# Mingqj/DFU3D

Measured on AMD Instinct MI355X. Metric: pseudo-box frames/sec (34k pts, 6 cams), higher is better.
Workload: dtype f64; 1 GPU; configs[1] with depth back-projection on (dense): 64 synthetic frames/GPU/step, 34720-pt sweep, 6 cams x 1600x900 depth + 8 instance masks (one bit-packed 1-byte word per pixel), 30-40 objects/scene; views_per_launch_chunk=192, streams=2, parallelism=frames sharded x1

## Files before the change

### dfu3d_amd/_lib.py

```python
import ctypes
import os
import re

from . import _build

c_void_p = ctypes.c_void_p
c_i32 = ctypes.c_int32
c_i64 = ctypes.c_int64
c_u64 = ctypes.c_uint64
c_f64 = ctypes.c_double

HEADER = os.path.join(_build.INCLUDE, "dfu3d.h")


class BinGeom(ctypes.Structure):
    _fields_ = [
        ("vsize_r", c_f64), ("vsize_t", c_f64), ("vsize_p", c_f64),
        ("rmin_r", c_f64), ("rmin_t", c_f64), ("rmin_p", c_f64),
        ("grid_r", c_i32), ("grid_t", c_i32), ("grid_p", c_i32),
        ("t_lo", c_i32), ("t_n", c_i32), ("p_lo", c_i32), ("p_n", c_i32),
        ("max_points_per_voxel", c_i32), ("max_voxels", c_i32),
        ("theta_min", c_f64), ("z_max", c_f64), ("depth_min", c_f64),
    ]

# ... 64 lines not shown
                                     _P]),
    "dfu3d_ballquery_fuse_joint": (c_i32, [_P, _P, _P, _P, _P, _P, _P, c_f64, c_i32, c_i64, _P, _P,
                                     _P]),
    "dfu3d_range_cluster": (c_i32, [_P, _P, _P, _P, c_i32, c_f64, c_f64, _P, _P, _P, _P, c_i64,
                                    _P]),
    "dfu3d_points_in_boxes_mask": (c_i32, [_P, c_i32, c_i32, _P, c_i32, _P, _P]),
    "dfu3d_gt_database": (c_i32, [_P, _P, _P, _P, c_i32, _P, _P, c_i64, _P, _P, _P, _P]),
    "dfu3d_boxes_bev": (c_i32, [_P, c_i32, _P, c_i32, _P, c_i32, _P]),
    "dfu3d_nms_bev": (c_i32, [_P, c_i32, ctypes.c_float, _P, _P, _P, _P]),
    "dfu3d_nms_normal_bev": (c_i32, [_P, c_i32, ctypes.c_float, _P, _P, _P, _P]),
    "dfu3d_boxes_bev_paired": (c_i32, [_P, _P, c_i32, _P, c_i32, _P]),
    "dfu3d_rotate_iou_eval": (c_i32, [_P, c_i32, _P, c_i32, _P, c_i32, _P]),
    "dfu3d_eval_overlaps": (c_i32, [c_i32, c_i32, _P, _P, _P, _P, _P, _P, _P, _P, c_i64, _P]),
    "dfu3d_eval_match_scores": (c_i32, [c_i32, c_i32, c_i32] + [_P] * 15 + [c_i32, c_i64, _P, _P, _P]),
    "dfu3d_eval_match_stats": (c_i32, [c_i32, c_i32, c_i32] + [_P] * 15 + [c_i32, _P, _P, c_i32, c_i32, _P, _P, _P]),
    "dfu3d_workspace_bytes": (c_i64, [c_i32, ctypes.POINTER(Sizes)]),
    "dfu3d_chain_workspace_bytes": (c_i64, [ctypes.POINTER(ChainCfg)]),
    "dfu3d_chain_workspace_init": (c_i32, [ctypes.POINTER(ChainCfg), _P, _P]),
    "dfu3d_pseudo_boxes": (c_i32, [ctypes.POINTER(ChainCfg)] + [_P] * 20),
    "dfu3d_la_sampling": (c_i32, [_P, c_i32, _P, c_i32, ctypes.c_float, ctypes.c_float, _P, _P, _P, c_i64, _P]),
    "dfu3d_selftest_classify": (c_i32, [_P, c_i32, c_i32, _P, c_i32, c_i64, ctypes.c_uint64, c_f64, c_f64, _P, _P, _P]),
    "dfu3d_selftest_backproject": (c_i32, [_P, c_i32, c_i32, c_i64, ctypes.c_uint64, c_f64, c_f64, _P, _P, _P]),
    "dfu3d_lshape_fit_ws_doubles": (c_i64, [c_i64, c_i32]),
    "dfu3d_lshape_fit": (c_i32, [_P, _P, _P, _P, _P, _P, c_i32, c_i32, _P, _P, _P, _P, _P,
                                 c_i32, c_f64, c_f64, _P, _P, _P, c_i32, _P, _P, _P, _P, c_i64,
                                 _P]),
}

_LIB = None


class Dfu3dError(RuntimeError):
    pass


def header_symbols():
    text = open(HEADER).read()
    text = re.sub(r"/\*.*?\*/", "", text, flags=re.S)
    return sorted(set(re.findall(r"\b(dfu3d_[a-z0-9_]+)\s*\(", text)))


def header_version():
    return int(re.search(r"#define\s+DFU3D_VERSION\s+(\d+)", open(HEADER).read()).group(1))


def lib():
# ... 43 lines not shown
```

### dfu3d_amd/csrc/fit_stage.hip

```cpp
#include "common.hpp"

namespace {
__device__ __forceinline__ int rl_i(int v, int l) { return __builtin_amdgcn_readlane(v, l); }
__device__ __forceinline__ double rl_d(double v, int l) {
  return __hiloint2double(__builtin_amdgcn_readlane(__double2hiint(v), l), __builtin_amdgcn_readlane(__double2loint(v), l));
}

constexpr int CT = 512;
constexpr int GRP = 32;
constexpr int BLK = 32;
constexpr int PAIR_SMALL = 32;
constexpr int GU = 4;
constexpr int SMALL_N = 4096;
constexpr int LARGE_N = 61440;
constexpr int LARGE_GRP = LARGE_N / GRP;
constexpr int GRID_NC_SMALL = 4096;
constexpr int GRID_NC_LARGE = 12288;

struct ParI {
  int *p;
  bool global;
  __device__ __forceinline__ int load(int i) const {
    return __hip_atomic_load(p + i, __ATOMIC_RELAXED, __HIP_MEMORY_SCOPE_AGENT);
  }
// ... 781 lines not shown
    const int slot = atomicAdd(n_rows, 1);
    if (slot < cap_rows) {
      double *o = rows + (size_t)slot * DFU3D_ROW_DOUBLES;
      o[0] = (double)v; o[1] = (double)jinst; o[2] = (double)kc;
      o[3] = (double)inst_class[s]; o[4] = alpha;
      o[5] = (double)inst_box[s * 4 + 0]; o[6] = (double)inst_box[s * 4 + 1];
      o[7] = (double)inst_box[s * 4 + 2]; o[8] = (double)inst_box[s * 4 + 3];
      o[9] = height; o[10] = width; o[11] = length;
      o[12] = rx; o[13] = ry; o[14] = rz; o[15] = rotation;
      o[16] = (double)inst_score[s]; o[17] = (double)m;
      o[18] = thb; o[19] = c1min; o[20] = c2min; o[21] = c1max; o[22] = c2max;
      o[23] = (double)root;
    } else {
      atomicOr(status, DFU3D_ST_ROW_OVERFLOW);
    }
  }
}

struct FitWs {
  int *counters;
  double *dsc;
  int *big_list;
  double *big_cost;
  int cap_q, cap_big;
};
__host__ __device__ inline int fit_cap_q(int cap_rows) { return 2 * cap_rows + 64; }
__host__ __device__ inline FitWs fit_ws_view(double *ws, int cap_rows, int cap_big) {
  FitWs w;
  w.cap_q = fit_cap_q(cap_rows);
  w.cap_big = cap_big;
  w.counters = (int *)ws;
  w.dsc = ws + 2;
  w.big_list = (int *)(w.dsc + (size_t)8 * w.cap_q);
  w.big_cost = w.dsc + (size_t)8 * w.cap_q + (cap_big / 2 + 1);
  return w;
}

constexpr int GK = 512;

__device__ __forceinline__ int rank_in(const int *roots, int nk, int L) {
  int lo = 0, hi = nk - 1;
  while (lo < hi) {
    const int mid = (lo + hi) >> 1;
    if (roots[mid] < L) lo = mid + 1; else hi = mid;
  }
  return (roots[lo] == L) ? lo : -1;
}

constexpr int GGU = 4;
__global__ __launch_bounds__(FT) void k_fit_gather(
    const double *__restrict__ px, const double *__restrict__ py,
    const double *__restrict__ pz, const int *__restrict__ label,
    const long long *__restrict__ seg_base, const int *__restrict__ seg_cnt,
    double *__restrict__ gsx, double *__restrict__ gsy, int *__restrict__ sroot,
    uint32_t *__restrict__ status, double *__restrict__ fit_ws, int cap_rows, int cap_big) {
  __shared__ int s_roots[GK];
  __shared__ int s_cnt[FW][GK];
// ... 181 lines not shown
struct FitAcc {
  double s1, s2, q1, q2;
  int n1, n2;
  __device__ __forceinline__ void clear() { s1 = s2 = q1 = q2 = 0.0; n1 = n2 = 0; }
  __device__ __forceinline__ void add(double x, double y, double ct, double st, double a0, double a1, double b0, double b1) {
    const double c1 = x * ct + y * st;
    const double c2 = x * (-st) + y * ct;
    const double d1 = fmin(fabs(a1 - c1), fabs(c1 - a0));
    const double d2 = fmin(fabs(b1 - c2), fabs(c2 - b0));
    if (d1 < d2) { s1 += d1; q1 = fma(d1, d1, q1); n1++; } else { s2 += d2; q2 = fma(d2, d2, q2); n2++; }
  }
  __device__ __forceinline__ void wave_reduce() {
    s1 = wave_sum_d(s1); s2 = wave_sum_d(s2); q1 = wave_sum_d(q1); q2 = wave_sum_d(q2);
    n1 = wave_sum_i(n1); n2 = wave_sum_i(n2);
  }
  __device__ __forceinline__ double cost(double &mag) const {
    double V1 = 0.0, V2 = 0.0, M1 = 0.0, M2 = 0.0;
    if (n1) { const double mu = s1 / (double)n1; M1 = q1 / (double)n1; V1 = -(M1 - mu * mu); }
    if (n2) { const double mu = s2 / (double)n2; M2 = q2 / (double)n2; V2 = -(M2 - mu * mu); }
    mag = M1 + M2;
    return V1 + V2;
  }
};
__device__ __forceinline__ double wave_exact_cost(const double *mx, const double *my, int m, double ct, double st) {
  const int lane = lane_id();
  double a0 = INFINITY, a1 = -INFINITY, b0 = INFINITY, b1 = -INFINITY;
  for (int i = lane; i < m; i += 64) {
    const double x = mx[i], y = my[i];
    const double c1 = x * ct + y * st;
    const double c2 = x * (-st) + y * ct;
    a0 = fmin(a0, c1); a1 = fmax(a1, c1);
    b0 = fmin(b0, c2); b1 = fmax(b1, c2);
  }
  a0 = wave_min_d(a0); a1 = wave_max_d(a1);
  b0 = wave_min_d(b0); b1 = wave_max_d(b1);
  double s1 = 0.0, s2 = 0.0;
  int n1 = 0, n2 = 0;
  for (int i = lane; i < m; i += 64) {
    const double x = mx[i], y = my[i];
    const double c1 = x * ct + y * st;
    const double c2 = x * (-st) + y * ct;
    const double d1 = fmin(fabs(a1 - c1), fabs(c1 - a0));
    const double d2 = fmin(fabs(b1 - c2), fabs(c2 - b0));
    if (d1 < d2) { s1 += d1; n1++; } else { s2 += d2; n2++; }
  }
  s1 = wave_sum_d(s1); s2 = wave_sum_d(s2);
// ... 150 lines not shown
      const double c1 = x * cos_s + y * sin_s;
      const double c2 = x * (-sin_s) + y * cos_s;
      a0 = c1; a1 = c1; b0 = c2; b1 = c2;
    }
    a0 = wave_min_d(a0); a1 = wave_max_d(a1);
    b0 = wave_min_d(b0); b1 = wave_max_d(b1);
    if (lane == 0) {
      const int s = (int)d[0], kc = (int)d[1], root = (int)d[2];
      const int v = s / max_inst, jinst = s - v * max_inst;
      emit_box(thb, sin_s, cos_s, a0, a1, b0, b1, d[5], s, v, jinst, kc, root, m, calib, inst_class,
               inst_is_car, inst_box, inst_score, car_aspect_max, cap_rows, rows, n_rows, status);
    }
  }
}

__global__ __launch_bounds__(FT, 8) void k_fit_medium(
    const double *__restrict__ gsx, const double *__restrict__ gsy, int max_inst,
    const ViewCalib *__restrict__ calib, const int *__restrict__ inst_class,
    const int *__restrict__ inst_is_car, const float *__restrict__ inst_box,
    const float *__restrict__ inst_score, int n_theta, double dtheta, double car_aspect_max,
    int cap_rows, double *__restrict__ rows, int *__restrict__ n_rows,
    uint32_t *__restrict__ status, double *__restrict__ fit_ws, int cap_big) {
  __shared__ double lx[LDS_MEMBERS], ly[LDS_MEMBERS];
  __shared__ double s_cost[MAXTH], s_mag[MAXTH], s_ct[MAXTH], s_st[MAXTH];
  __shared__ double s_ext[FW][4];
  const FitWs W = fit_ws_view(fit_ws, cap_rows, cap_big);
  const int nq = min(W.counters[0], W.cap_q);
  const int wave = threadIdx.x >> 6, lane = lane_id();
  if (threadIdx.x < MAXTH) {
    const double theta = (double)threadIdx.x * dtheta;
    s_ct[threadIdx.x] = cos(theta);
    s_st[threadIdx.x] = sin(theta);
  }
  __shared__ int s_item;
  while (true) {
    __syncthreads();
    if (wave == 0) {
      const int ticket = atomicAdd(&W.counters[3], 1);
      if (lane == 0) s_item = ticket >> 6;
    }
    __syncthreads();
    const int e = s_item;
    if (e >= nq) break;
    const double *d = W.dsc + (size_t)8 * e;
    const int m = (int)d[3];
    if (m <= 64 || m > LDS_MEMBERS) continue;
    __syncthreads();
    const long long P = (long long)d[4];
    for (int i = threadIdx.x; i < m; i += FT) { lx[i] = gsx[P + i]; ly[i] = gsy[P + i]; }
    __syncthreads();
    const double *mx = lx;
    const double *my = ly;
    for (int th0 = 2 * wave; th0 < n_theta; th0 += 2 * FW) {
      const int th1 = min(th0 + 1, n_theta - 1);
      const double ct0 = s_ct[th0], st0 = s_st[th0], ct1 = s_ct[th1], st1 = s_st[th1];
      double a0 = INFINITY, a1 = -INFINITY, b0 = INFINITY, b1 = -INFINITY;
      double e0 = INFINITY, e1 = -INFINITY, f0 = INFINITY, f1 = -INFINITY;
      for (int i = lane; i < m; i += 64) {
        const double x = mx[i], y = my[i];
        double c1 = x * ct0 + y * st0;
        double c2 = x * (-st0) + y * ct0;
        a0 = min_raw_d(a0, c1); a1 = max_raw_d(a1, c1);
        b0 = min_raw_d(b0, c2); b1 = max_raw_d(b1, c2);
        c1 = x * ct1 + y * st1;
        c2 = x * (-st1) + y * ct1;
        e0 = min_raw_d(e0, c1); e1 = max_raw_d(e1, c1);
        f0 = min_raw_d(f0, c2); f1 = max_raw_d(f1, c2);
      }
      a0 = wave_min_d(a0); a1 = wave_max_d(a1); b0 = wave_min_d(b0); b1 = wave_max_d(b1);
      e0 = wave_min_d(e0); e1 = wave_max_d(e1); f0 = wave_min_d(f0); f1 = wave_max_d(f1);
      FitAcc A, B;
      A.clear(); B.clear();
      for (int i = lane; i < m; i += 64) {
        const double x = mx[i], y = my[i];
        A.add(x, y, ct0, st0, a0, a1, b0, b1);
        B.add(x, y, ct1, st1, e0, e1, f0, f1);
      }
      A.wave_reduce(); B.wave_reduce();
      double magA, magB;
      const double cA = A.cost(magA), cB = B.cost(magB);
      if (lane == 0) { s_cost[th0] = cA; s_mag[th0] = magA; s_cost[th1] = cB; s_mag[th1] = magB; }
    }
    __syncthreads();
    double magmax = 0.0;
    for (int th = 0; th < n_theta; th++) { const double g = s_mag[th]; if (g > magmax) magmax = g; }
    const int best = wave_pick_heading(s_cost, n_theta, magmax, mx, my, m, s_ct, s_st);
    const double thb = (double)best * dtheta;
    const double sin_s = sin(thb), cos_s = cos(thb);
    {
      double a0 = INFINITY, a1 = -INFINITY, b0 = INFINITY, b1 = -INFINITY;
      for (int i = threadIdx.x; i < m; i += FT) {
        const double x = mx[i], y = my[i];
        const double c1 = x * cos_s + y * sin_s;
        const double c2 = x * (-sin_s) + y * cos_s;
        a0 = fmin(a0, c1); a1 = fmax(a1, c1);
        b0 = fmin(b0, c2); b1 = fmax(b1, c2);
      }
      a0 = wave_min_d(a0); a1 = wave_max_d(a1);
      b0 = wave_min_d(b0); b1 = wave_max_d(b1);
      if (lane == 0) { s_ext[wave][0] = a0; s_ext[wave][1] = a1; s_ext[wave][2] = b0; s_ext[wave][3] = b1; }
    }
    __syncthreads();
    if (threadIdx.x == 0) {
      double c1min = s_ext[0][0], c1max = s_ext[0][1], c2min = s_ext[0][2], c2max = s_ext[0][3];
      for (int w = 1; w < FW; w++) {
        c1min = fmin(c1min, s_ext[w][0]); c1max = fmax(c1max, s_ext[w][1]);
        c2min = fmin(c2min, s_ext[w][2]); c2max = fmax(c2max, s_ext[w][3]);
      }
      const int s = (int)d[0], kc = (int)d[1], root = (int)d[2];
      const int v = s / max_inst, jinst = s - v * max_inst;
      emit_box(thb, sin_s, cos_s, c1min, c1max, c2min, c2max, d[5], s, v, jinst, kc, root, m, calib,
               inst_class, inst_is_car, inst_box, inst_score, car_aspect_max, cap_rows, rows,
               n_rows, status);
    }
  }
}

constexpr int BIGC_T = 512, BIGC_WAVES = BIGC_T / 64, BIGC_HPW = 2, BIGC_HB = BIGC_WAVES * BIGC_HPW;
constexpr int BIGC_CH = 4096;
constexpr int BIGC_LONG = 16384, BIGC_MID = 6144;
__global__ __launch_bounds__(BIGC_T) void k_fit_big_cost(const double *__restrict__ gsx,
                                                         const double *__restrict__ gsy, int n_theta,
                                                         double dtheta, double *__restrict__ fit_ws,
                                                         int cap_rows, int cap_big) {
  __shared__ double lx[BIGC_CH], ly[BIGC_CH];
  __shared__ double s_ct[MAXTH], s_st[MAXTH];
  __shared__ int s_item;
  const FitWs W = fit_ws_view(fit_ws, cap_rows, cap_big);
  const int nbig = min(W.counters[1], cap_big);
  if (nbig == 0) return;
  if (threadIdx.x < MAXTH) {
    const double theta = (double)threadIdx.x * dtheta;
    s_ct[threadIdx.x] = cos(theta);
    s_st[threadIdx.x] = sin(theta);
  }
  const int wave = threadIdx.x >> 6, lane = lane_id();
  const int nb = (n_theta + BIGC_HB - 1) / BIGC_HB;
  const int items = nbig * nb;
  while (true) {
    __syncthreads();
    if (wave == 0) {
      const int ticket = atomicAdd(&W.counters[2], 1);
      if (lane == 0) s_item = ticket >> 6;
    }
    __syncthreads();
    const int ticket_item = s_item;
    if (ticket_item >= 3 * items) break;
    const int round = ticket_item / items;
    const int item = ticket_item - round * items;
    const int c = item / nb, tb = (item - c * nb) * BIGC_HB;
    const double *dsc = W.dsc + (size_t)8 * W.big_list[c];
    const int m = (int)dsc[3];
    if ((m > BIGC_LONG ? 0 : (m > BIGC_MID ? 1 : 2)) != round) continue;
    const double *mx = gsx + (long long)dsc[4], *my = gsy + (long long)dsc[4];
    int th[BIGC_HPW];
    double ct[BIGC_HPW], st[BIGC_HPW], nst[BIGC_HPW];
#pragma unroll
    for (int h = 0; h < BIGC_HPW; h++) {
      th[h] = tb + wave * BIGC_HPW + h;
      const int tc = min(th[h], n_theta - 1);
      ct[h] = s_ct[tc]; st[h] = s_st[tc]; nst[h] = -st[h];
    }
    double a0[BIGC_HPW], a1[BIGC_HPW], b0[BIGC_HPW], b1[BIGC_HPW];
#pragma unroll
    for (int h = 0; h < BIGC_HPW; h++) { a0[h] = INFINITY; a1[h] = -INFINITY; b0[h] = INFINITY; b1[h] = -INFINITY; }
    for (int c0 = 0; c0 < m; c0 += BIGC_CH) {
      const int cm = min(BIGC_CH, m - c0);
      __syncthreads();
      for (int i = threadIdx.x; i < cm; i += BIGC_T) { lx[i] = mx[c0 + i]; ly[i] = my[c0 + i]; }
      __syncthreads();
      for (int i = lane; i < cm; i += 64) {
        const double x = lx[i], y = ly[i];
#pragma unroll
        for (int h = 0; h < BIGC_HPW; h++) {
          const double c1 = x * ct[h] + y * st[h];
          const double c2 = x * nst[h] + y * ct[h];
          a0[h] = min_raw_d(a0[h], c1); a1[h] = max_raw_d(a1[h], c1);
          b0[h] = min_raw_d(b0[h], c2); b1[h] = max_raw_d(b1[h], c2);
        }
      }
    }
#pragma unroll
    for (int h = 0; h < BIGC_HPW; h++) {
      a0[h] = wave_min_d(a0[h]); a1[h] = wave_max_d(a1[h]);
      b0[h] = wave_min_d(b0[h]); b1[h] = wave_max_d(b1[h]);
    }
    FitAcc A[BIGC_HPW];
#pragma unroll
    for (int h = 0; h < BIGC_HPW; h++) A[h].clear();
    for (int c0 = 0; c0 < m; c0 += BIGC_CH) {
      const int cm = min(BIGC_CH, m - c0);
      __syncthreads();
      for (int i = threadIdx.x; i < cm; i += BIGC_T) { lx[i] = mx[c0 + i]; ly[i] = my[c0 + i]; }
      __syncthreads();
      for (int i = lane; i < cm; i += 64) {
        const double x = lx[i], y = ly[i];
#pragma unroll
        for (int h = 0; h < BIGC_HPW; h++) A[h].add(x, y, ct[h], st[h], a0[h], a1[h], b0[h], b1[h]);
      }
    }
#pragma unroll
    for (int h = 0; h < BIGC_HPW; h++) {
      A[h].wave_reduce();
      double mag;
      const double cst = A[h].cost(mag);
      if (lane == 0 && th[h] < n_theta) {
        W.big_cost[(size_t)c * MAXTH + th[h]] = cst;
        if (mag > 0.0) atomicMax((unsigned long long *)(W.dsc + (size_t)8 * W.big_list[c] + 7), (unsigned long long)__double_as_longlong(mag));
// ... 35 lines not shown
    const double c1 = x * cos_s + y * sin_s;
    const double c2 = x * (-sin_s) + y * cos_s;
    a0 = fmin(a0, c1); a1 = fmax(a1, c1);
    b0 = fmin(b0, c2); b1 = fmax(b1, c2);
  }
  a0 = wave_min_d(a0); a1 = wave_max_d(a1);
  b0 = wave_min_d(b0); b1 = wave_max_d(b1);
  if (lane == 0) { s_ext[wave][0] = a0; s_ext[wave][1] = a1; s_ext[wave][2] = b0; s_ext[wave][3] = b1; }
  __syncthreads();
  if (threadIdx.x == 0) {
    double c1min = s_ext[0][0], c1max = s_ext[0][1], c2min = s_ext[0][2], c2max = s_ext[0][3];
    for (int w = 1; w < FW; w++) {
      c1min = fmin(c1min, s_ext[w][0]); c1max = fmax(c1max, s_ext[w][1]);
      c2min = fmin(c2min, s_ext[w][2]); c2max = fmax(c2max, s_ext[w][3]);
    }
    const int v = s / max_inst, jinst = s - v * max_inst;
    emit_box(thb, sin_s, cos_s, c1min, c1max, c2min, c2max, zmax, s, v, jinst, kc, root, m, calib,
             inst_class, inst_is_car, inst_box, inst_score, car_aspect_max, cap_rows, rows, n_rows,
             status);
  }
  }
}

}

extern "C" int dfu3d_range_cluster(const double *px, const double *py, const int64_t *seg_base,
                                   const int32_t *seg_cnt, int32_t S, double R0, double Rd,
                                   int32_t *label, double *sx, double *sy, int32_t *si,
                                   int64_t pool_cap, void *stream) {
  DFU3D_CLEAR_STALE_ERROR();
  if (!px || !py || !seg_base || !seg_cnt || !label || !sx || !sy || !si) return DFU3D_EINVAL;
  if (S <= 0 || pool_cap <= 0 || !(R0 > 0.0) || !(Rd >= 0.0)) return DFU3D_EINVAL;
  hipLaunchKernelGGL((k_range_cluster_grid<GRID_NC_SMALL, 0, 1024>), dim3(CL_CLASSES * S), dim3(1024), 0,
                     (hipStream_t)stream, px, py, (const long long *)seg_base, seg_cnt, R0, Rd,
                     label, sx, sy, si, (long long)pool_cap, 0, 0x7FFFFFFF);
  DFU3D_LAUNCH_CHECK();
  hipLaunchKernelGGL((k_range_cluster_grid<GRID_NC_LARGE, GRID_NC_SMALL, 1024>), dim3(CL_CLASSES * S), dim3(1024), 0,
                     (hipStream_t)stream, px, py, (const long long *)seg_base, seg_cnt, R0, Rd,
                     label, sx, sy, si, (long long)pool_cap, 0, 0x7FFFFFFF);
  DFU3D_LAUNCH_CHECK();
  hipLaunchKernelGGL(k_range_cluster_small, dim3(S), dim3(CT), 0, (hipStream_t)stream, px, py,
                     (const long long *)seg_base, seg_cnt, R0, Rd, label, sx, sy, si,
                     (long long)pool_cap);
  DFU3D_LAUNCH_CHECK();
  hipLaunchKernelGGL(k_range_cluster_large, dim3(S), dim3(CT), 0, (hipStream_t)stream, px, py,
                     (const long long *)seg_base, seg_cnt, R0, Rd, label, sx, sy, si,
                     (long long)pool_cap);
  DFU3D_LAUNCH_CHECK();
  return DFU3D_OK;
}


extern "C" int64_t dfu3d_lshape_fit_ws_doubles(int64_t pool_cap, int32_t cap_rows) {
  if (pool_cap <= 0 || cap_rows <= 0) return DFU3D_EINVAL;
  const int64_t cap_big = pool_cap / LDS_MEMBERS + 1;
  return 2 + (int64_t)8 * fit_cap_q(cap_rows) + (cap_big / 2 + 1) + cap_big * MAXTH;
}

extern "C" int dfu3d_lshape_fit(const double *px, const double *py, const double *pz,
                                const int32_t *label, const int64_t *seg_base,
                                const int32_t *seg_cnt, int32_t S, int32_t max_inst,
                                const float *calib, const int32_t *inst_class,
                                const int32_t *inst_is_car, const float *inst_box,
                                const float *inst_score, int32_t n_theta, double dtheta,
                                double car_aspect_max, double *sx, double *sy, int32_t *sroot,
                                int32_t cap_rows, double *rows, int32_t *n_rows,
                                uint32_t *status, double *fit_ws, int64_t pool_cap,
                                void *stream) {
  DFU3D_CLEAR_STALE_ERROR();
  if (!px || !py || !pz || !label || !seg_base || !seg_cnt || !calib || !inst_class ||
      !inst_is_car || !inst_box || !inst_score || !sx || !sy || !sroot || !rows || !n_rows ||
      !status || !fit_ws)
    return DFU3D_EINVAL;
  if (S <= 0 || max_inst <= 0 || cap_rows <= 0 || n_theta <= 0 || pool_cap <= 0) return DFU3D_EINVAL;
  if (n_theta > MAXTH) return DFU3D_ERANGE;
  hipStream_t st = (hipStream_t)stream;
  const int cap_big = (int)(pool_cap / LDS_MEMBERS + 1);
  const ViewCalib *vc = (const ViewCalib *)calib;
  if (dfu3d_fill_small_async(fit_ws, 16, nullptr, 0, nullptr, 0, st) != hipSuccess) return DFU3D_ELAUNCH;
  hipLaunchKernelGGL(k_fit_gather, dim3(3 * S), dim3(FT), 0, st, px, py, pz, label,
                     (const long long *)seg_base, seg_cnt, sx, sy, sroot, status, fit_ws,
                     cap_rows, cap_big);
  DFU3D_LAUNCH_CHECK();
  const int cap_q = fit_cap_q(cap_rows);
  const int g_tiny = cap_q / 4 + 1 < 2048 ? cap_q / 4 + 1 : 2048;
  hipLaunchKernelGGL(k_fit_tiny, dim3(g_tiny), dim3(256), 0, st, sx, sy, max_inst, vc, inst_class,
                     inst_is_car, inst_box, inst_score, n_theta, dtheta, car_aspect_max, cap_rows,
                     rows, n_rows, status, fit_ws, cap_big);
  DFU3D_LAUNCH_CHECK();
  hipLaunchKernelGGL(k_fit_medium, dim3(cap_q < 2048 ? cap_q : 2048), dim3(FT), 0, st, sx, sy, max_inst,
                     vc, inst_class, inst_is_car, inst_box, inst_score, n_theta, dtheta,
                     car_aspect_max, cap_rows, rows, n_rows, status, fit_ws, cap_big);
  DFU3D_LAUNCH_CHECK();
  const long long bi = (long long)cap_big * ((n_theta + BIGC_HB - 1) / BIGC_HB);
  const int g2 = (int)(bi < 2048 ? bi : 2048);
  hipLaunchKernelGGL(k_fit_big_cost, dim3(g2), dim3(BIGC_T), 0, st, sx, sy, n_theta, dtheta,
                     fit_ws, cap_rows, cap_big);
  DFU3D_LAUNCH_CHECK();
  hipLaunchKernelGGL(k_fit_big_box, dim3(cap_big < 2048 ? cap_big : 2048), dim3(FT), 0, st, sx, sy, max_inst,
                     vc, inst_class, inst_is_car, inst_box, inst_score,
                     n_theta, dtheta, car_aspect_max, cap_rows, rows, n_rows, status, fit_ws,
                     cap_big);
  DFU3D_LAUNCH_CHECK();
  return DFU3D_OK;
}

extern "C" int dfu3d_version(void) { return DFU3D_VERSION; }

extern "C" const char *dfu3d_strerror(int code) {
  switch (code) {
    case DFU3D_OK: return "ok";
    case DFU3D_EINVAL: return "invalid argument";
    case DFU3D_ELAUNCH: return "kernel launch failed";
    case DFU3D_ERANGE: return "size exceeds a compiled-in limit";
    default: return "unknown error";
  }
// ... 2 lines not shown
```

### dfu3d_amd/stages.py

```python
import ctypes
import math

import numpy as np
from dataclasses import dataclass

import torch

from . import _lib
from ._lib import BinGeom, Dfu3dError

CALIB_FLOATS = 48
ROW_DOUBLES = 24
MAX_INST = 32

BP_BIN, BP_AMB, BP_MARK, BP_VOX, BP_REPAIR, BP_ALL = 1, 2, 4, 8, 16, 31
MASK_BYTES = 0
RF_SHADOW, RF_FLAGS, RF_RESOLVE, RF_COMPACT, RF_ALL = 1, 2, 4, 8, 15

ST_POOL_OVERFLOW = 1
ST_VOX_OVERFLOW = 2
ST_ROW_OVERFLOW = 4
ST_BIN_RANGE = 8
ST_VOX_PTS_OVERFLOW = 16
ST_VOXEL_RANGE = 32
# ... 476 lines not shown
    scratch = torch.zeros(SELFTEST_SCRATCH_BYTES // 4, dtype=torch.float32, device=device)
    out = torch.zeros(4, dtype=torch.int64, device=device)
    rc = _lib.lib().dfu3d_selftest_classify(_chk(cal, "calib", torch.float32, numel=CALIB_FLOATS), int(H), int(W),
                                            ctypes.byref(geom), int(key_axis), int(n), int(seed), float(d_lo),
                                            float(d_hi), _chk(scratch, "scratch", torch.float32),
                                            _chk(out, "out", torch.int64, numel=4), _stream())
    _lib.check(rc, "dfu3d_selftest_classify")
    t, u, w, k = out.cpu().tolist()
    return {"tried": t, "undecided": u, "wrong": w, "kept": k}


def selftest_backproject(calib_record, H, W, n, seed=1, d_lo=0.5, d_hi=120.0, device="cuda:0"):
    cal = torch.as_tensor(np.asarray(calib_record, np.float32).reshape(CALIB_FLOATS)).to(device).contiguous()
    scratch = torch.zeros(32, dtype=torch.float32, device=device)
    out = torch.zeros(1, dtype=torch.float64, device=device)
    rc = _lib.lib().dfu3d_selftest_backproject(_chk(cal, "calib", torch.float32, numel=CALIB_FLOATS), int(H), int(W),
                                               int(n), int(seed), float(d_lo), float(d_hi),
                                               _chk(scratch, "scratch", torch.float32, numel=32),
                                               _chk(out, "out", torch.float64, numel=1), _stream())
    _lib.check(rc, "dfu3d_selftest_backproject")
    return float(out.item())


def range_cluster(px, py, seg_base, seg_cnt, S, R0, Rd, label, pool_cap, sx=None, sy=None, si=None):
    dev = px.device
    sx = sx if sx is not None else torch.empty(pool_cap, dtype=torch.float64, device=dev)
    sy = sy if sy is not None else torch.empty(pool_cap, dtype=torch.float64, device=dev)
    si = si if si is not None else torch.empty(3 * pool_cap, dtype=torch.int32, device=dev)
    rc = _lib.lib().dfu3d_range_cluster(
        _chk(px, "px", torch.float64, numel=pool_cap), _chk(py, "py", torch.float64, numel=pool_cap),
        _chk(seg_base, "seg_base", torch.int64, numel=S),
        _chk(seg_cnt, "seg_cnt", torch.int32, numel=S), S, float(R0), float(Rd),
        _chk(label, "label", torch.int32, numel=pool_cap),
        _chk(sx, "sx", torch.float64, numel=pool_cap), _chk(sy, "sy", torch.float64, numel=pool_cap),
        _chk(si, "si", torch.int32, numel=3 * pool_cap), pool_cap, _stream())
    _lib.check(rc, "dfu3d_range_cluster")


def lshape_fit(px, py, pz, label, seg_base, seg_cnt, S, max_inst, calib, inst_class,
               inst_is_car, inst_box, inst_score, n_theta, dtheta, car_aspect_max, sx, sy,
               sroot, cap_rows, rows, n_rows, status, pool_cap, fit_ws=None):
    nws = int(_lib.lib().dfu3d_lshape_fit_ws_doubles(pool_cap, cap_rows))
    if fit_ws is None:
        fit_ws = torch.empty(nws, dtype=torch.float64, device=px.device)
    if S % max_inst:
        raise Dfu3dError("S must be V*max_inst")
# ... 25 lines not shown
```

### include/dfu3d.h

```cpp
#ifndef DFU3D_H
#define DFU3D_H

#include <stddef.h>
#include <stdint.h>

#ifdef __cplusplus
extern "C" {
#endif

#define DFU3D_VERSION 150
#define DFU3D_CALIB_FLOATS 48
#define DFU3D_ROW_DOUBLES 24
#define DFU3D_TABLE_ENTRY_BYTES 28
#define DFU3D_MAX_INST 32

#define DFU3D_OK 0
#define DFU3D_EINVAL (-1)
#define DFU3D_ELAUNCH (-2)
#define DFU3D_ERANGE (-3)

#define DFU3D_ST_POOL_OVERFLOW 1u
#define DFU3D_ST_VOX_OVERFLOW 2u
#define DFU3D_ST_ROW_OVERFLOW 4u
#define DFU3D_ST_BIN_RANGE 8u
// ... 202 lines not shown
int dfu3d_selftest_classify(const float *calib, int32_t H, int32_t W, const dfu3d_bin_geom *geom,
                            int32_t key_axis, int64_t n, uint64_t seed, double d_lo, double d_hi,
                            void *scratch, uint64_t *out4, void *stream);
int dfu3d_selftest_backproject(const float *calib, int32_t H, int32_t W, int64_t n, uint64_t seed,
                               double d_lo, double d_hi, void *scratch64, double *out1, void *stream);

int dfu3d_range_cluster(const double *px, const double *py,
                        const int64_t *seg_base, const int32_t *seg_cnt,
                        int32_t S, double R0, double Rd, int32_t *label,
                        double *sx, double *sy, int32_t *si, int64_t pool_cap,
                        void *stream);

int64_t dfu3d_lshape_fit_ws_doubles(int64_t pool_cap, int32_t cap_rows);
int dfu3d_lshape_fit(const double *px, const double *py, const double *pz,
                     const int32_t *label, const int64_t *seg_base,
                     const int32_t *seg_cnt, int32_t S, int32_t max_inst,
                     const float *calib, const int32_t *inst_class,
                     const int32_t *inst_is_car, const float *inst_box,
                     const float *inst_score, int32_t n_theta, double dtheta,
                     double car_aspect_max, double *sx, double *sy,
                     int32_t *sroot, int32_t cap_rows, double *rows,
                     int32_t *n_rows, uint32_t *status, double *fit_ws,
                     int64_t pool_cap, void *stream);

typedef struct dfu3d_chain_cfg {
  int32_t V, H, W, max_inst, cap_n, cap_vox, cap_rows;
  int32_t dense, apply_fov, fov_h, fov_w, stat_filter;
  int32_t bounds_h, bounds_w;
  int32_t mask_format, reserved0;
  double stat_voxel;
  int64_t pool_cap;
  double plane_max_hs, plane_range, plane_offset;
  int32_t ransac_trials, nb_points;
  uint64_t ransac_seed;
  double fuse_C, R0, Rd;
  int32_t n_theta, stat_nb_neighbors;
  double dtheta, car_aspect_max, stat_std_ratio;
  dfu3d_bin_geom geom;
} dfu3d_chain_cfg;
int64_t dfu3d_chain_workspace_bytes(const dfu3d_chain_cfg *cfg);
int dfu3d_chain_workspace_init(const dfu3d_chain_cfg *cfg, void *workspace, void *stream);
int dfu3d_pseudo_boxes(const dfu3d_chain_cfg *cfg, const float *points,
                       const int32_t *pt_off, const int32_t *view_frame,
                       const float *calib, const void *masks,
                       const int32_t *n_inst, const float *depth,
                       const int64_t *view_key, const double *plane_in,
// ... 11 lines not shown
```

Measured before the change: 10190 frames/s.

## Prune L-shape extent search to convex-hull candidates and precompute big-cluster extents

Before the per-heading L-shape cost pass, each cluster now gets an approximate 16-direction convex polygon, and only points outside its conservatively shrunk interior are kept as candidates for the min/max projections at each heading. Medium clusters compute extents once from these candidates in LDS rather than rescanning every point per heading pair. Big clusters get a new k_fit_big_ext kernel that slices them across blocks and merges extents through ordered-key atomicMax into a workspace array, replacing the full chunked extent scan inside k_fit_big_cost. This adds a launch, more workspace, and float-precision hull tests with an epsilon margin, and it ships a selftest entry point to check exactness.

```diff
diff --git a/dfu3d_amd/_lib.py b/dfu3d_amd/_lib.py
--- a/dfu3d_amd/_lib.py
+++ b/dfu3d_amd/_lib.py
@@ -110,6 +110,7 @@
     "dfu3d_selftest_classify": (c_i32, [_P, c_i32, c_i32, _P, c_i32, c_i64, ctypes.c_uint64, c_f64, c_f64, _P, _P, _P]),
     "dfu3d_selftest_backproject": (c_i32, [_P, c_i32, c_i32, c_i64, ctypes.c_uint64, c_f64, c_f64, _P, _P, _P]),
     "dfu3d_lshape_fit_ws_doubles": (c_i64, [c_i64, c_i32]),
+    "dfu3d_selftest_fit_extents": (c_i32, [_P, _P, _P, c_i32, _P, _P, c_i32, _P, _P, _P]),
     "dfu3d_lshape_fit": (c_i32, [_P, _P, _P, _P, _P, _P, c_i32, c_i32, _P, _P, _P, _P, _P,
                                  c_i32, c_f64, c_f64, _P, _P, _P, c_i32, _P, _P, _P, _P, c_i64,
                                  _P]),
diff --git a/dfu3d_amd/csrc/fit_stage.hip b/dfu3d_amd/csrc/fit_stage.hip
--- a/dfu3d_amd/csrc/fit_stage.hip
+++ b/dfu3d_amd/csrc/fit_stage.hip
@@ -827,6 +827,7 @@
   double *dsc;
   int *big_list;
   double *big_cost;
+  double *big_ext;
   int cap_q, cap_big;
 };
 __host__ __device__ inline int fit_cap_q(int cap_rows) { return 2 * cap_rows + 64; }
@@ -838,6 +839,7 @@
   w.dsc = ws + 2;
   w.big_list = (int *)(w.dsc + (size_t)8 * w.cap_q);
   w.big_cost = w.dsc + (size_t)8 * w.cap_q + (cap_big / 2 + 1);
+  w.big_ext = w.big_cost + (size_t)cap_big * MAXTH;
   return w;
 }
 
@@ -1065,6 +1067,190 @@
     return V1 + V2;
   }
 };
+constexpr int HULL_AX = 8, HULL_K = 2 * HULL_AX;
+constexpr int HULL_EDGE = 5;
+static_assert(FW * HULL_K * 8 <= MAXTH * 8 && HULL_K * HULL_EDGE <= MAXTH, "hull scratch is one MAXTH-double array");
+
+__device__ __forceinline__ double shfl_d(double v, int src) {
+  const int lo = __shfl(__double2loint(v), src, 64), hi = __shfl(__double2hiint(v), src, 64);
+  return __hiloint2double(hi, lo);
+}
+__constant__ float HULL_C[HULL_AX] = {1.0f, 0.92387953f, 0.70710678f, 0.38268343f, 0.0f, -0.38268343f, -0.70710678f,
+                                      -0.92387953f};
+__constant__ float HULL_S[HULL_AX] = {0.0f, 0.38268343f, 0.70710678f, 0.92387953f, 1.0f, 0.92387953f, 0.70710678f,
+                                      0.38268343f};
+template <int T, int AP>
+__device__ __forceinline__ int hull_build(const double *mx, const double *my, int m, double *scr, double *scr2) {
+  constexpr int NW = T / 64;
+  static_assert(NW <= FW && FW * 8 >= HULL_K * 4, "scratch is sized for FW waves");
+  static_assert(HULL_AX % AP == 0, "whole passes");
+  const int wave = threadIdx.x >> 6, lane = lane_id();
+  float *kv = (float *)scr;
+  int *ki = (int *)scr + NW * HULL_K;
+  const double x0 = mx[0], y0 = my[0];
+  double r = 0.0;
+#pragma unroll 1
+  for (int k0 = 0; k0 < HULL_AX; k0 += AP) {
+    float bv[2 * AP];
+    int bi[2 * AP];
+#pragma unroll
+    for (int a = 0; a < 2 * AP; a++) { bv[a] = -INFINITY; bi[a] = -1; }
+    for (int i = threadIdx.x; i < m; i += T) {
+      const double x = mx[i], y = my[i];
+      if (k0 == 0) r = fmax(r, fabs(x) + fabs(y));
+      const float fx = (float)(x - x0), fy = (float)(y - y0);
+#pragma unroll
+      for (int a = 0; a < AP; a++) {
+        const float p = fx * HULL_C[k0 + a] + fy * HULL_S[k0 + a];
+        if (p > bv[a]) { bv[a] = p; bi[a] = i; }
+        if (-p > bv[AP + a]) { bv[AP + a] = -p; bi[AP + a] = i; }
+      }
+    }
+#pragma unroll
+    for (int a = 0; a < 2 * AP; a++) {
+#pragma unroll
+      for (int msk = 32; msk >= 1; msk >>= 1) {
+        const float ov = __shfl_xor(bv[a], msk, 64);
+        const int oi = __shfl_xor(bi[a], msk, 64);
+        if (ov > bv[a] || (ov == bv[a] && oi > bi[a])) { bv[a] = ov; bi[a] = oi; }
+      }
+    }
+    if (lane == 0) {
+#pragma unroll
+      for (int a = 0; a < AP; a++) {
+        kv[wave * HULL_K + k0 + a] = bv[a]; ki[wave * HULL_K + k0 + a] = bi[a];
+        kv[wave * HULL_K + HULL_AX + k0 + a] = bv[AP + a]; ki[wave * HULL_K + HULL_AX + k0 + a] = bi[AP + a];
+      }
+    }
+  }
+  r = wave_max_d(r);
+  if (lane == 0) scr2[wave] = r;
+  __syncthreads();
+  if (wave == 0) {
+    const int k = lane & (HULL_K - 1);
+    double R = 0.0;
+    for (int w = 0; w < NW; w++) R = fmax(R, scr2[w]);
+    float v = kv[k];
+    int id = ki[k];
+    for (int w = 1; w < NW; w++) {
+      const float ov = kv[w * HULL_K + k];
+      const int oi = ki[w * HULL_K + k];
+      if (ov > v || (ov == v && oi > id)) { v = ov; id = oi; }
+    }
+    const bool ok = __ballot(id < 0) == 0ull;
+    const double vx = mx[max(id, 0)], vy = my[max(id, 0)];
+    const int nb = (lane & ~(HULL_K - 1)) | ((k + 1) & (HULL_K - 1));
+    const double nx = shfl_d(vx, nb), ny = shfl_d(vy, nb);
+    const double ox = shfl_d(vx, lane & ~(HULL_K - 1)), oy = shfl_d(vy, lane & ~(HULL_K - 1));
+    const bool real = !(nx == vx && ny == vy);
+    const double ex = nx - vx, ey = ny - vy;
+    double area = (vx - ox) * (ny - oy) - (vy - oy) * (nx - ox);
+#pragma unroll
+    for (int msk = HULL_K / 2; msk >= 1; msk >>= 1) area += shfl_xor_d(area, msk);
+    const int nreal = __popcll(__ballot(real) & ((1ull << HULL_K) - 1ull));
+    const int ne = (ok && nreal >= 3 && area > 0.0) ? HULL_K : 0;
+    if (lane < HULL_K) {
+      double *e = scr + HULL_EDGE * lane;
+      e[0] = vx; e[1] = vy; e[2] = ex; e[3] = ey;
+      e[4] = real ? 0x1p-40 * R * sqrt(ex * ex + ey * ey) : -INFINITY;
+    }
+    if (lane == 0) scr2[FW] = (double)ne;
+  }
+  __syncthreads();
+  return (int)scr2[FW];
+}
+__device__ __forceinline__ bool hull_inside(double x, double y, const double *E, int ne) {
+  bool in = ne > 0;
+  for (int k = 0; k < ne; k++) {
+    const double *e = E + HULL_EDGE * k;
+    const double cr = e[2] * (y - e[1]) - e[3] * (x - e[0]);
+    in = in & (cr > e[4]);
+  }
+  return in;
+}
+constexpr int HULL_AP_LDS = 2;
+__device__ __forceinline__ int fit_candidates_lds(const double *lx, const double *ly, int m, double *scr, double *scr2,
+                                                  unsigned short *cand, int *s_nc) {
+  if (threadIdx.x == 0) *s_nc = 0;
+  const int ne = hull_build<FT, HULL_AP_LDS>(lx, ly, m, scr, scr2);
+  const int lane = lane_id();
+  for (int b = 0; b < m; b += FT) {
+    const int i = b + threadIdx.x;
+    bool c = false;
+    if (i < m) c = !hull_inside(lx[i], ly[i], scr, ne);
+    const unsigned long long bal = __ballot(c);
+    int base = 0;
+    if (lane == 0 && bal) base = atomicAdd(s_nc, __popcll(bal));
+    base = __shfl(base, 0, 64);
+    if (c) cand[base + __popcll(bal & ((1ull << lane) - 1ull))] = (unsigned short)i;
+  }
+  __syncthreads();
+  return *s_nc;
+}
+__device__ __forceinline__ unsigned long long ord_key(double v) {
+  const unsigned long long u = (unsigned long long)__double_as_longlong(v);
+  return (u >> 63) ? ~u : (u | 0x8000000000000000ull);
+}
+__device__ __forceinline__ double ord_val(unsigned long long k) {
+  return __longlong_as_double((long long)((k >> 63) ? (k & 0x7FFFFFFFFFFFFFFFull) : ~k));
+}
+__device__ __forceinline__ void ext_from_keys(const unsigned long long *k, double &a0, double &a1, double &b0,
+                                              double &b1) {
+  a0 = ord_val(~k[0]); a1 = ord_val(k[1]); b0 = ord_val(~k[2]); b1 = ord_val(k[3]);
+}
+__device__ __forceinline__ bool cand_extents(const double *lx, const double *ly, const unsigned short *cand, int nc,
+                                             int n_theta, const double *ctab, const double *stab, int &th, double &a0,
+                                             double &a1, double &b0, double &b1) {
+  static_assert(16 * FW >= MAXTH, "a lane per heading");
+  const int wave = threadIdx.x >> 6, lane = lane_id();
+  const int g = lane >> 4;
+  th = 16 * wave + (lane & 15);
+  a0 = INFINITY; a1 = -INFINITY; b0 = INFINITY; b1 = -INFINITY;
+  if (16 * wave >= n_theta) return false;
+  const int tc = min(th, n_theta - 1);
+  const double ct = ctab[tc], st = stab[tc];
+  for (int j = g; j < nc; j += 4) {
+    const int i = cand[j];
+    const double x = lx[i], y = ly[i];
+    const double c1 = x * ct + y * st;
+    const double c2 = x * (-st) + y * ct;
+    a0 = min_raw_d(a0, c1); a1 = max_raw_d(a1, c1);
+    b0 = min_raw_d(b0, c2); b1 = max_raw_d(b1, c2);
+  }
+#pragma unroll
+  for (int msk = 16; msk <= 32; msk <<= 1) {
+    a0 = min_raw_d(a0, shfl_xor_d(a0, msk)); a1 = max_raw_d(a1, shfl_xor_d(a1, msk));
+    b0 = min_raw_d(b0, shfl_xor_d(b0, msk)); b1 = max_raw_d(b1, shfl_xor_d(b1, msk));
+  }
+  return g == 0 && th < n_theta;
+}
+__device__ __forceinline__ int medium_extents(const double *lx, const double *ly, int m, int n_theta, const double *ctab,
+                                              const double *stab, unsigned short *cand, double *scr, double *scr2,
+                                              int *s_nc, double *ext4) {
+  const int nc = fit_candidates_lds(lx, ly, m, scr, scr2, cand, s_nc);
+  int th;
+  double a0, a1, b0, b1;
+  const bool mine = cand_extents(lx, ly, cand, nc, n_theta, ctab, stab, th, a0, a1, b0, b1);
+  __syncthreads();
+  if (mine) { ext4[4 * th] = a0; ext4[4 * th + 1] = a1; ext4[4 * th + 2] = b0; ext4[4 * th + 3] = b1; }
+  __syncthreads();
+  return nc;
+}
+__device__ __forceinline__ int slice_extents(const double *lx, const double *ly, int m, int n_theta, const double *ctab,
+                                             const double *stab, unsigned short *cand, double *scr, double *scr2,
+                                             int *s_nc, unsigned long long *keys) {
+  const int nc = fit_candidates_lds(lx, ly, m, scr, scr2, cand, s_nc);
+  int th;
+  double a0, a1, b0, b1;
+  if (cand_extents(lx, ly, cand, nc, n_theta, ctab, stab, th, a0, a1, b0, b1)) {
+    unsigned long long *k = keys + 4 * th;
+    atomicMax(k + 0, ~ord_key(a0)); atomicMax(k + 1, ord_key(a1));
+    atomicMax(k + 2, ~ord_key(b0)); atomicMax(k + 3, ord_key(b1));
+  }
+  return nc;
+}
+constexpr int BIGX_SLY = 16;
+
 __device__ __forceinline__ double wave_exact_cost(const double *mx, const double *my, int m, double ct, double st) {
   const int lane = lane_id();
   double a0 = INFINITY, a1 = -INFINITY, b0 = INFINITY, b1 = -INFINITY;
@@ -1261,8 +1447,11 @@
     int cap_rows, double *__restrict__ rows, int *__restrict__ n_rows,
     uint32_t *__restrict__ status, double *__restrict__ fit_ws, int cap_big) {
   __shared__ double lx[LDS_MEMBERS], ly[LDS_MEMBERS];
-  __shared__ double s_cost[MAXTH], s_mag[MAXTH], s_ct[MAXTH], s_st[MAXTH];
+  __shared__ __align__(8) unsigned short s_cand[LDS_MEMBERS];
+  __shared__ double s_cost[MAXTH], s_ct[MAXTH], s_st[MAXTH];
   __shared__ double s_ext[FW][4];
+  __shared__ double s_magw[FW];
+  __shared__ int s_nc;
   const FitWs W = fit_ws_view(fit_ws, cap_rows, cap_big);
   const int nq = min(W.counters[0], W.cap_q);
   const int wave = threadIdx.x >> 6, lane = lane_id();
@@ -1283,46 +1472,47 @@
     if (e >= nq) break;
     const double *d = W.dsc + (size_t)8 * e;
     const int m = (int)d[3];
-    if (m <= 64 || m > LDS_MEMBERS) continue;
+    if (m > LDS_MEMBERS) {
+      const int bi = (int)d[6];
+      static_assert(MAXTH * 4 <= FT, "one key per thread");
+      if (bi >= 0 && threadIdx.x < MAXTH * 4)
+        ((unsigned long long *)W.big_ext)[(size_t)bi * MAXTH * 4 + threadIdx.x] = 0ull;
+      continue;
+    }
+    if (m <= 64) continue;
     __syncthreads();
     const long long P = (long long)d[4];
     for (int i = threadIdx.x; i < m; i += FT) { lx[i] = gsx[P + i]; ly[i] = gsy[P + i]; }
     __syncthreads();
     const double *mx = lx;
     const double *my = ly;
+    const double *ext4 = (const double *)s_cand;
+    medium_extents(lx, ly, m, n_theta, s_ct, s_st, s_cand, s_cost, &s_ext[0][0], &s_nc, (double *)s_cand);
+    double magw = 0.0;
     for (int th0 = 2 * wave; th0 < n_theta; th0 += 2 * FW) {
       const int th1 = min(th0 + 1, n_theta - 1);
       const double ct0 = s_ct[th0], st0 = s_st[th0], ct1 = s_ct[th1], st1 = s_st[th1];
-      double a0 = INFINITY, a1 = -INFINITY, b0 = INFINITY, b1 = -INFINITY;
-      double e0 = INFINITY, e1 = -INFINITY, f0 = INFINITY, f1 = -INFINITY;
-      for (int i = lane; i < m; i += 64) {
-        const double x = mx[i], y = my[i];
-        double c1 = x * ct0 + y * st0;
-        double c2 = x * (-st0) + y * ct0;
-        a0 = min_raw_d(a0, c1); a1 = max_raw_d(a1, c1);
-        b0 = min_raw_d(b0, c2); b1 = max_raw_d(b1, c2);
-        c1 = x * ct1 + y * st1;
-        c2 = x * (-st1) + y * ct1;
-        e0 = min_raw_d(e0, c1); e1 = max_raw_d(e1, c1);
-        f0 = min_raw_d(f0, c2); f1 = max_raw_d(f1, c2);
-      }
-      a0 = wave_min_d(a0); a1 = wave_max_d(a1); b0 = wave_min_d(b0); b1 = wave_max_d(b1);
-      e0 = wave_min_d(e0); e1 = wave_max_d(e1); f0 = wave_min_d(f0); f1 = wave_max_d(f1);
+      double e[8];
+#pragma unroll
+      for (int q = 0; q < 4; q++) { e[q] = ext4[4 * th0 + q]; e[4 + q] = ext4[4 * th1 + q]; }
       FitAcc A, B;
       A.clear(); B.clear();
       for (int i = lane; i < m; i += 64) {
         const double x = mx[i], y = my[i];
-        A.add(x, y, ct0, st0, a0, a1, b0, b1);
-        B.add(x, y, ct1, st1, e0, e1, f0, f1);
+        A.add(x, y, ct0, st0, e[0], e[1], e[2], e[3]);
+        B.add(x, y, ct1, st1, e[4], e[5], e[6], e[7]);
       }
       A.wave_reduce(); B.wave_reduce();
       double magA, magB;
       const double cA = A.cost(magA), cB = B.cost(magB);
-      if (lane == 0) { s_cost[th0] = cA; s_mag[th0] = magA; s_cost[th1] = cB; s_mag[th1] = magB; }
-    }
+      if (magA > magw) magw = magA;
+      if (magB > magw) magw = magB;
+      if (lane == 0) { s_cost[th0] = cA; s_cost[th1] = cB; }
+    }
+    if (lane == 0) s_magw[wave] = magw;
     __syncthreads();
     double magmax = 0.0;
-    for (int th = 0; th < n_theta; th++) { const double g = s_mag[th]; if (g > magmax) magmax = g; }
+    for (int w = 0; w < FW; w++) { const double g = s_magw[w]; if (g > magmax) magmax = g; }
     const int best = wave_pick_heading(s_cost, n_theta, magmax, mx, my, m, s_ct, s_st);
     const double thb = (double)best * dtheta;
     const double sin_s = sin(thb), cos_s = cos(thb);
@@ -1358,6 +1548,36 @@
 constexpr int BIGC_T = 512, BIGC_WAVES = BIGC_T / 64, BIGC_HPW = 2, BIGC_HB = BIGC_WAVES * BIGC_HPW;
 constexpr int BIGC_CH = 4096;
 constexpr int BIGC_LONG = 16384, BIGC_MID = 6144;
+__global__ __launch_bounds__(FT) void k_fit_big_ext(const double *__restrict__ gsx, const double *__restrict__ gsy,
+                                                    int n_theta, double dtheta, double *__restrict__ fit_ws,
+                                                    int cap_rows, int cap_big) {
+  __shared__ double lx[LDS_MEMBERS], ly[LDS_MEMBERS];
+  __shared__ unsigned short s_cand[LDS_MEMBERS];
+  __shared__ double s_scr[MAXTH], s_scr2[FW + 1];
+  __shared__ double s_ct[MAXTH], s_st[MAXTH];
+  __shared__ int s_nc;
+  const FitWs W = fit_ws_view(fit_ws, cap_rows, cap_big);
+  const int nbig = min(W.counters[1], cap_big);
+  if (threadIdx.x < MAXTH) {
+    const double theta = (double)threadIdx.x * dtheta;
+    s_ct[threadIdx.x] = cos(theta);
+    s_st[threadIdx.x] = sin(theta);
+  }
+  for (int c = blockIdx.x; c < nbig; c += gridDim.x) {
+    const double *dsc = W.dsc + (size_t)8 * W.big_list[c];
+    const int m = (int)dsc[3];
+    const long long P = (long long)dsc[4];
+    for (int j0 = blockIdx.y * LDS_MEMBERS; j0 < m; j0 += gridDim.y * LDS_MEMBERS) {
+      const int cm = min(LDS_MEMBERS, m - j0);
+      __syncthreads();
+      for (int i = threadIdx.x; i < cm; i += FT) { lx[i] = gsx[P + j0 + i]; ly[i] = gsy[P + j0 + i]; }
+      __syncthreads();
+      slice_extents(lx, ly, cm, n_theta, s_ct, s_st, s_cand, s_scr, s_scr2, &s_nc,
+                    (unsigned long long *)W.big_ext + (size_t)c * MAXTH * 4);
+    }
+  }
+}
+
 __global__ __launch_bounds__(BIGC_T) void k_fit_big_cost(const double *__restrict__ gsx,
                                                          const double *__restrict__ gsy, int n_theta,
                                                          double dtheta, double *__restrict__ fit_ws,
@@ -1402,27 +1622,9 @@
     }
     double a0[BIGC_HPW], a1[BIGC_HPW], b0[BIGC_HPW], b1[BIGC_HPW];
 #pragma unroll
-    for (int h = 0; h < BIGC_HPW; h++) { a0[h] = INFINITY; a1[h] = -INFINITY; b0[h] = INFINITY; b1[h] = -INFINITY; }
-    for (int c0 = 0; c0 < m; c0 += BIGC_CH) {
-      const int cm = min(BIGC_CH, m - c0);
-      __syncthreads();
-      for (int i = threadIdx.x; i < cm; i += BIGC_T) { lx[i] = mx[c0 + i]; ly[i] = my[c0 + i]; }
-      __syncthreads();
-      for (int i = lane; i < cm; i += 64) {
-        const double x = lx[i], y = ly[i];
-#pragma unroll
-        for (int h = 0; h < BIGC_HPW; h++) {
-          const double c1 = x * ct[h] + y * st[h];
-          const double c2 = x * nst[h] + y * ct[h];
-          a0[h] = min_raw_d(a0[h], c1); a1[h] = max_raw_d(a1[h], c1);
-          b0[h] = min_raw_d(b0[h], c2); b1[h] = max_raw_d(b1[h], c2);
-        }
-      }
-    }
-#pragma unroll
     for (int h = 0; h < BIGC_HPW; h++) {
-      a0[h] = wave_min_d(a0[h]); a1[h] = wave_max_d(a1[h]);
-      b0[h] = wave_min_d(b0[h]); b1[h] = wave_max_d(b1[h]);
+      ext_from_keys((const unsigned long long *)W.big_ext + ((size_t)c * MAXTH + min(th[h], n_theta - 1)) * 4, a0[h],
+                    a1[h], b0[h], b1[h]);
     }
     FitAcc A[BIGC_HPW];
 #pragma unroll
@@ -1504,6 +1706,64 @@
   }
 }
 
+__global__ __launch_bounds__(FT) void k_selftest_fit_extents(const double *__restrict__ px, const double *__restrict__ py,
+                                                             const long long *__restrict__ off, int n_clusters,
+                                                             const double *__restrict__ ctab,
+                                                             const double *__restrict__ stab, int n_theta,
+                                                             unsigned long long *__restrict__ keys,
+                                                             int *__restrict__ ncand) {
+  __shared__ double lx[LDS_MEMBERS], ly[LDS_MEMBERS];
+  __shared__ __align__(8) unsigned short s_cand[LDS_MEMBERS];
+  __shared__ double s_scr[MAXTH], s_scr2[FW + 1];
+  __shared__ double s_ct[MAXTH], s_st[MAXTH];
+  __shared__ int s_nc;
+  if (threadIdx.x < n_theta) { s_ct[threadIdx.x] = ctab[threadIdx.x]; s_st[threadIdx.x] = stab[threadIdx.x]; }
+  for (int c = blockIdx.x; c < n_clusters; c += gridDim.x) {
+    const long long P = off[c];
+    const int m = (int)(off[c + 1] - P);
+    for (int j0 = blockIdx.y * LDS_MEMBERS; j0 < m; j0 += gridDim.y * LDS_MEMBERS) {
+      const int cm = min(LDS_MEMBERS, m - j0);
+      __syncthreads();
+      for (int i = threadIdx.x; i < cm; i += FT) { lx[i] = px[P + j0 + i]; ly[i] = py[P + j0 + i]; }
+      __syncthreads();
+      unsigned long long *kc = keys + (size_t)c * n_theta * 4;
+      int nc;
+      if (m <= LDS_MEMBERS) {
+        nc = medium_extents(lx, ly, cm, n_theta, s_ct, s_st, s_cand, s_scr, s_scr2, &s_nc, (double *)s_cand);
+        const double *ext4 = (const double *)s_cand;
+        for (int q = threadIdx.x; q < 4 * n_theta; q += FT) kc[q] = (q & 1) ? ord_key(ext4[q]) : ~ord_key(ext4[q]);
+      } else {
+        nc = slice_extents(lx, ly, cm, n_theta, s_ct, s_st, s_cand, s_scr, s_scr2, &s_nc, kc);
+      }
+      if (threadIdx.x == 0) atomicAdd(ncand + c, nc);
+    }
+  }
+}
+__global__ void k_selftest_fit_decode(unsigned long long *keys, long long n) {
+  for (long long i = blockIdx.x * (long long)blockDim.x + threadIdx.x; i < n; i += (long long)gridDim.x * blockDim.x) {
+    const unsigned long long k = keys[i];
+    keys[i] = (unsigned long long)__double_as_longlong((i & 1) ? ord_val(k) : ord_val(~k));
+  }
+}
+
+}
+
+extern "C" int dfu3d_selftest_fit_extents(const double *px, const double *py, const int64_t *offsets,
+                                          int32_t n_clusters, const double *ct, const double *st, int32_t n_theta,
+                                          double *ext, int32_t *ncand, void *stream) {
+  DFU3D_CLEAR_STALE_ERROR();
+  if (!px || !py || !offsets || !ct || !st || !ext || !ncand || n_clusters <= 0 || n_theta <= 0) return DFU3D_EINVAL;
+  if (n_theta > MAXTH) return DFU3D_ERANGE;
+  hipStream_t hs = (hipStream_t)stream;
+  const long long nk = (long long)n_clusters * n_theta * 4;
+  if (hipMemsetAsync(ext, 0, (size_t)nk * 8, hs) != hipSuccess) return DFU3D_ELAUNCH;
+  if (hipMemsetAsync(ncand, 0, (size_t)n_clusters * 4, hs) != hipSuccess) return DFU3D_ELAUNCH;
+  hipLaunchKernelGGL(k_selftest_fit_extents, dim3(n_clusters < 1024 ? n_clusters : 1024, BIGX_SLY), dim3(FT), 0, hs, px,
+                     py, (const long long *)offsets, n_clusters, ct, st, n_theta, (unsigned long long *)ext, ncand);
+  DFU3D_LAUNCH_CHECK();
+  hipLaunchKernelGGL(k_selftest_fit_decode, dim3(256), dim3(256), 0, hs, (unsigned long long *)ext, nk);
+  DFU3D_LAUNCH_CHECK();
+  return DFU3D_OK;
 }
 
 extern "C" int dfu3d_range_cluster(const double *px, const double *py, const int64_t *seg_base,
@@ -1536,7 +1796,7 @@
 extern "C" int64_t dfu3d_lshape_fit_ws_doubles(int64_t pool_cap, int32_t cap_rows) {
   if (pool_cap <= 0 || cap_rows <= 0) return DFU3D_EINVAL;
   const int64_t cap_big = pool_cap / LDS_MEMBERS + 1;
-  return 2 + (int64_t)8 * fit_cap_q(cap_rows) + (cap_big / 2 + 1) + cap_big * MAXTH;
+  return 2 + (int64_t)8 * fit_cap_q(cap_rows) + (cap_big / 2 + 1) + cap_big * MAXTH * 5;
 }
 
 extern "C" int dfu3d_lshape_fit(const double *px, const double *py, const double *pz,
@@ -1574,6 +1834,9 @@
                      vc, inst_class, inst_is_car, inst_box, inst_score, n_theta, dtheta,
                      car_aspect_max, cap_rows, rows, n_rows, status, fit_ws, cap_big);
   DFU3D_LAUNCH_CHECK();
+  hipLaunchKernelGGL(k_fit_big_ext, dim3(cap_big < 256 ? cap_big : 256, BIGX_SLY), dim3(FT), 0, st, sx, sy, n_theta,
+                     dtheta, fit_ws, cap_rows, cap_big);
+  DFU3D_LAUNCH_CHECK();
   const long long bi = (long long)cap_big * ((n_theta + BIGC_HB - 1) / BIGC_HB);
   const int g2 = (int)(bi < 2048 ? bi : 2048);
   hipLaunchKernelGGL(k_fit_big_cost, dim3(g2), dim3(BIGC_T), 0, st, sx, sy, n_theta, dtheta,
diff --git a/dfu3d_amd/stages.py b/dfu3d_amd/stages.py
--- a/dfu3d_amd/stages.py
+++ b/dfu3d_amd/stages.py
@@ -522,6 +522,19 @@
     return float(out.item())
 
 
+def selftest_fit_extents(px, py, offsets, ct, st):
+    C, n_theta = offsets.numel() - 1, ct.numel()
+    ext = torch.full((C, n_theta, 4), float("nan"), dtype=torch.float64, device=px.device)
+    ncand = torch.full((C,), -1, dtype=torch.int32, device=px.device)
+    rc = _lib.lib().dfu3d_selftest_fit_extents(
+        _chk(px, "px", torch.float64), _chk(py, "py", torch.float64, numel=px.numel()),
+        _chk(offsets, "offsets", torch.int64), C, _chk(ct, "ct", torch.float64),
+        _chk(st, "st", torch.float64, numel=n_theta), n_theta, _chk(ext, "ext", torch.float64),
+        _chk(ncand, "ncand", torch.int32), _stream())
+    _lib.check(rc, "dfu3d_selftest_fit_extents")
+    return ext, ncand
+
+
 def range_cluster(px, py, seg_base, seg_cnt, S, R0, Rd, label, pool_cap, sx=None, sy=None, si=None):
     dev = px.device
     sx = sx if sx is not None else torch.empty(pool_cap, dtype=torch.float64, device=dev)
diff --git a/include/dfu3d.h b/include/dfu3d.h
--- a/include/dfu3d.h
+++ b/include/dfu3d.h
@@ -248,6 +248,10 @@
                      int32_t *sroot, int32_t cap_rows, double *rows,
                      int32_t *n_rows, uint32_t *status, double *fit_ws,
                      int64_t pool_cap, void *stream);
+
+int dfu3d_selftest_fit_extents(const double *px, const double *py, const int64_t *offsets,
+                               int32_t n_clusters, const double *ct, const double *st,
+                               int32_t n_theta, double *ext, int32_t *ncand, void *stream);
 
 typedef struct dfu3d_chain_cfg {
   int32_t V, H, W, max_inst, cap_n, cap_vox, cap_rows;
```

Measured after the change: 10170 frames/s (median of 3 runs). About the same (-0.2%).
